# SysSec-KAIST/LTESniffer

Measured on AMD Instinct MI355X. Metric: subframes/s (20 MHz, 150 RNTIs), higher is better.
Workload: dtype f32+int16

## Files before the change

ltesniffer_amd/csrc/kernels/lsn_dsp.h:

```cpp
#pragma once
#include "lsn_dev.h"
#include "lsn_fft_map.h"

__device__ __forceinline__ cf32 cmul(cf32 a, cf32 b) { cf32 c; c.r = a.r * b.r - a.i * b.i; c.i = a.r * b.i + a.i * b.r; return c; }
__device__ __forceinline__ cf32 cmulconj(cf32 a, cf32 b) { cf32 c; c.r = a.r * b.r + a.i * b.i; c.i = a.i * b.r - a.r * b.i; return c; }
__device__ __forceinline__ float cabs2(cf32 a) { return a.r * a.r + a.i * a.i; }

template <int R, int S, int LG>
__device__ __forceinline__ void fft_twiddles(cf32* tw, const cf32* __restrict__ W, int low)
{
#pragma unroll
  for (int q = 0; q < R; q++)
#pragma unroll
    for (int m = 0; m < (1 << q); m++) tw[(1 << q) - 1 + m] = W[lsn_fft_twiddle(low + (m << S), S + q, LG)];
}
template <int R>
__device__ __forceinline__ void fft_butterflies(cf32* e, const cf32* tw)
{
#pragma unroll
  for (int q = 0; q < R; q++) {
#pragma unroll
    for (int j = 0; j < (1 << R); j++) {
      if (j & (1 << q)) continue;
      cf32 v = cmul(e[j + (1 << q)], tw[(1 << q) - 1 + (j & ((1 << q) - 1))]);
      cf32 uu = e[j];
      e[j].r = uu.r + v.r; e[j].i = uu.i + v.i;
      e[j + (1 << q)].r = uu.r - v.r; e[j + (1 << q)].i = uu.i - v.i;
    }
  }
}
template <int R, int S, int LG, int NB>
__device__ __forceinline__ void fft_pass(cf32* a, const cf32* __restrict__ W, int tid)
{
  constexpr int G = 1 << R, NG = NB << (LG - R);
#pragma unroll
  for (int u = 0; u < (NG + LSN_FFT_THREADS - 1) / LSN_FFT_THREADS; u++) {
    const int gg = tid + LSN_FFT_THREADS * u;
    if (gg < NG) {
      const int r = NB == 1 ? 0 : gg >> (LG - R), g = gg & ((1 << (LG - R)) - 1), base = lsn_fft_base(g, S, R);
      const int at = lsn_fft_store(r, base, LG);
      cf32 e[G], tw[G - 1];
#pragma unroll
      for (int j = 0; j < G; j++) e[j] = a[at ^ lsn_fft_slot(j << S)];
      fft_twiddles<R, S, LG>(tw, W, base & ((1 << S) - 1));
      fft_butterflies<R>(e, tw);
#pragma unroll
      for (int j = 0; j < G; j++) a[at ^ lsn_fft_slot(j << S)] = e[j];
    }
  }
}
template <int R, int LG>
__device__ __forceinline__ void fft_last_pass(cf32* a, const cf32* __restrict__ W, cf32* __restrict__ out, float* pw, int nre, int dc, int tid)
{
  constexpr int G = 1 << R, S = LG - R, NG = 1 << S, U = (NG + LSN_FFT_THREADS - 1) / LSN_FFT_THREADS;
  cf32 e[U][G], tw[U][G - 1];
#pragma unroll
  for (int u = 0; u < U; u++) {
    const int g = tid + LSN_FFT_THREADS * u;
    if (g < NG) {
      const int at = lsn_fft_store(0, g, LG);
#pragma unroll
      for (int j = 0; j < G; j++) e[u][j] = a[at ^ lsn_fft_slot(j << S)];
      fft_twiddles<R, S, LG>(tw[u], W, g);
    }
  }
  if (pw) __syncthreads();
#pragma unroll
  for (int u = 0; u < U; u++) {
    const int g = tid + LSN_FFT_THREADS * u;
    if (g < NG) {
      fft_butterflies<R>(e[u], tw[u]);
#pragma unroll
      for (int j = 0; j < G; j++) {
        const int k = lsn_fft_carrier(g + (j << S), 1 << LG, nre, dc);
        if (k >= 0) {
          out[k] = e[u][j];
          if (pw) pw[k] = e[u][j].r * e[u][j].r + e[u][j].i * e[u][j].i;
        }
      }
    }
  }
}
template <int LG, int NB, typename Load>
__device__ __forceinline__ void fft_run(const LsnCellDev& c, cf32* a, Load load, cf32* __restrict__ out, float* pw, int dc, int tid)
{
  constexpr int M = 1 << LG, N = NB * M;
  const cf32* __restrict__ W = c.twiddle;
  const int nre = (int)c.nre;
  if (tid < N / 8) {
    cf32 x[8], e[8], tw[7];
#pragma unroll
    for (int jj = 0; jj < 8; jj++) x[jj] = load(lsn_fft_first_sample(tid, jj, N));
#pragma unroll
    for (int j = 0; j < 8; j++) e[j] = x[lsn_fft_brev3(j)];
    fft_twiddles<3, 0, LG>(tw, W, 0);
    fft_butterflies<3>(e, tw);
    int r, g;
    lsn_fft_first_group(tid, NB, LG, &r, &g);
    const int at = lsn_fft_store(r, 8 * g, LG);
#pragma unroll
    for (int j = 0; j < 8; j++) a[at ^ lsn_fft_slot(j)] = e[j];
  }
  __syncthreads();
  constexpr int R1 = LG >= 6 ? 3 : LG - 3, S2 = 3 + R1, R2 = LG - S2 >= 3 ? 3 : LG - S2, S3 = S2 + R2, R3 = LG - S3;
  static_assert(LG >= 7 && LG <= 11 && R2 >= 1 && R3 >= 0 && R3 <= 2, "pass plan");
  static_assert(R1 == 3 && (R3 == 0 || R2 == 3), "pass plan");
  fft_pass<R1, 3, LG, NB>(a, W, tid);
  __syncthreads();
  if constexpr (R3 > 0) {
    fft_pass<R2, S2, LG, NB>(a, W, tid);
    __syncthreads();
  }
  constexpr int RL = R3 > 0 ? R3 : R2, SL = LG - RL;
  if constexpr (NB == 1) {
    fft_last_pass<RL, LG>(a, W, out, pw, nre, dc, tid);
  } else {
    fft_pass<RL, SL, LG, NB>(a, W, tid);
    __syncthreads();
    const cf32* __restrict__ T = c.twiddle3;
    float p[6];
#pragma unroll
    for (int it = 0; it < 6; it++) {
      const int k = tid + LSN_FFT_THREADS * it;
      if (k < nre) {
        const int bin = lsn_fft_carrier_bin(k, N, nre, dc), kq = bin & (M - 1);
        int b2 = 2 * bin;
        b2 = b2 >= N ? b2 - N : b2;
// ... 59 lines not shown
```

ltesniffer_amd/csrc/kernels/lsn_fft_map.h:

```cpp
#pragma once
#include <stdint.h>
#ifndef LSN_HD
#ifdef __HIPCC__
#define LSN_HD __host__ __device__ __forceinline__
#else
#define LSN_HD static inline
#endif
#endif

#define LSN_FFT_THREADS 256

LSN_HD int lsn_fft_radix(int lgM, int s) { return (s == 0 || lgM - s >= 3) ? 3 : lgM - s; }

LSN_HD int lsn_fft_first_sample(int t, int jj, int N) { return t + (N >> 3) * jj; }
LSN_HD int lsn_fft_brev3(int j) { return ((j & 1) << 2) | (j & 2) | ((j >> 2) & 1); }
LSN_HD void lsn_fft_first_group(int t, int nb, int lgM, int* r, int* g)
{
  const int tt = nb == 3 ? t / 3 : t;
  *r = nb == 3 ? t - 3 * tt : 0;
#if defined(__has_builtin) && __has_builtin(__builtin_bitreverse32)
  *g = (int)(__builtin_bitreverse32((uint32_t)tt) >> (35 - lgM));
#else
  int b = 0;
  for (int k = 0; k < lgM - 3; k++) b |= ((tt >> k) & 1) << (lgM - 4 - k);
  *g = b;
#endif
}

LSN_HD int lsn_fft_groups(int nb, int lgM, int R) { return nb << (lgM - R); }
LSN_HD int lsn_fft_base(int g, int s, int R) { return ((g >> s) << (s + R)) | (g & ((1 << s) - 1)); }
LSN_HD int lsn_fft_twiddle(int pos, int stage, int lgM) { return pos << (lgM - stage - 1); }

LSN_HD int lsn_fft_slot(int i) { return i ^ ((i >> 3) & 0x1C) ^ ((i >> 5) & 2) ^ ((i >> 7) & 0xF); }
LSN_HD int lsn_fft_block_key(int r) { return (0x1A20 >> (5 * r)) & 31; }
LSN_HD int lsn_fft_store(int r, int i, int lgM) { return (r << lgM) | (lsn_fft_slot(i) ^ lsn_fft_block_key(r)); }
LSN_HD int lsn_fft_lds_slots(int N) { return N; }

LSN_HD int lsn_fft_carrier(int bin, int N, int nre, int dc)
{
  const int hf = nre >> 1;
  if (bin >= N - hf) return bin - (N - hf);
  if (bin >= dc && bin < dc + hf) return bin - dc + hf;
  return -1;
}
LSN_HD int lsn_fft_carrier_bin(int k, int N, int nre, int dc) { return k < (nre >> 1) ? N - (nre >> 1) + k : k - (nre >> 1) + dc; }
LSN_HD void lsn_fft_last_owner(int bin, int lgM, int R, int* t, int* u, int* j)
{
  const int g = bin & ((1 << (lgM - R)) - 1);
  *j = bin >> (lgM - R);
  *t = g & (LSN_FFT_THREADS - 1);
  *u = g >> 8;
}
```

ltesniffer_amd/csrc/kernels/stage_a.hip:

```cpp
#include "lsn_dsp.h"
#include <algorithm>
#include <type_traits>
#include <cstdlib>

#define SQRT2F 1.41421356237309504880f

__device__ __forceinline__ void ofdm_rb_power(const LsnCellDev& c, const float* pw, float* __restrict__ rbp_part, int sf, int l, int tid)
{
  __syncthreads();
  if (tid < (int)c.nof_prb) {
    const float4* q = (const float4*)(pw + tid * 12);
    const float4 q0 = q[0], q1 = q[1], q2 = q[2];
    const float v[12] = {q0.x, q0.y, q0.z, q0.w, q1.x, q1.y, q1.z, q1.w, q2.x, q2.y, q2.z, q2.w};
    float s = 0.0f;
    for (int k = 0; k < 12; k++) s = s + v[k];
    rbp_part[((size_t)sf * 14 + l) * 128 + tid] = s / 12.0f;
  }
}
__global__ __launch_bounds__(256) void k_ofdm(LsnCellDev c, const cf32* __restrict__ iq, const uint32_t* __restrict__ dphi_sf,
                                              cf32* __restrict__ grid, float* __restrict__ rbp_part)
{
  extern __shared__ __attribute__((aligned(16))) unsigned char smem[];
  const int N = (int)c.N, tid = threadIdx.x;
  cf32* a = (cf32*)smem;
  const int nsym = (int)c.nsym;
  const int blk = blockIdx.x, l = blk % nsym, rx = (blk / nsym) % (int)c.nof_rx, sf = blk / (nsym * (int)c.nof_rx);
  const int cp0 = 160 * N / 2048, cp1 = 144 * N / 2048;
  const int slot = l / 7, ls = l % 7;
  const int pos = c.cp ? l * (N + N / 4) + N / 4 : slot * (cp0 + 6 * cp1 + 7 * N) + cp0 + ls * (N + cp1);
  const cf32* in = iq + ((size_t)sf * c.iq_nant + rx) * c.sflen + pos;
  const uint32_t dphi = dphi_sf ? dphi_sf[sf] : 0u;
  const int nre = (int)c.nre;
  cf32* out = grid + (((size_t)sf * c.nof_rx + rx) * 14 + l) * nre;
  auto load = [&](int n) {
    cf32 x = in[n];
    if (dphi != 0u) {
      uint32_t ph = (uint32_t)(pos + n) * dphi;
      cf32 rot = cmul(c.nco_coarse[ph >> 20], c.nco_fine[(ph >> 10) & 1023u]);
      x = cmul(x, rot);
    }
    return x;
  };
  float* pw = (rbp_part && rx == 0) ? (float*)smem : nullptr;
  lsn_symbol_fft(c, a, load, out, pw, 1, tid);
  if (pw) ofdm_rb_power(c, pw, rbp_part, sf, l, tid);
}

void lsn_launch_ofdm(const LsnCellDev& c, const cf32* iq, const uint32_t* dphi, cf32* grid, uint32_t nsf, hipStream_t s, float* rbp_part)
{
  size_t lds = sizeof(cf32) * lsn_fft_lds_slots((int)c.N);
  LSN_LAUNCH(k_ofdm, dim3(nsf * c.nof_rx * c.nsym), dim3(256), lds, s, c, iq, dphi, grid, rbp_part);
}

__device__ __forceinline__ int crs_koff(const LsnCellDev& c, int port, int s)
{
  int v = (port == 0) ? ((s & 1) ? 3 : 0) : (port == 1) ? ((s & 1) ? 0 : 3) : (port == 2) ? 3 * s : 3 + 3 * s;
  return (v + (int)(c.id % 6)) % 6;
}

__global__ __launch_bounds__(256) void k_chest(LsnCellDev c, const cf32* __restrict__ grid, const uint32_t* __restrict__ sf_idx_arr,
                                               cf32* __restrict__ ce, float* __restrict__ raw)
{
  extern __shared__ __attribute__((aligned(16))) unsigned char smem[];
  const int nre = (int)c.nre, nref = (int)c.nref, tid = threadIdx.x;
  const int P = (int)c.nof_ports, A = (int)c.nof_rx;
  const int blk = blockIdx.x, p = blk % P, rx = (blk / P) % A, sf = blk / (P * A);
  cf32* ls = (cf32*)smem;
  cf32* sm = ls + 4 * nref;
  float* part = (float*)(sm + 4 * nref);
  const int S = p < 2 ? 4 : 2;
  const int nsl = (int)c.nslot, nsym = (int)c.nsym;
  const int sym[4] = {p < 2 ? 0 : 1, p < 2 ? nsl - 3 : nsl + 1, nsl, 2 * nsl - 3};
  const cf32* g = grid + ((size_t)sf * A + rx) * 14 * nre;
  const cf32* crs = c.crs + ((size_t)sf_idx_arr[sf] * P + p) * 4 * nref;
  const int n4 = S * nref;
  for (int i = tid; i < n4; i += 256) {
    int s = i / nref, m = i - s * nref;
    ls[i] = cmulconj(g[sym[s] * nre + 6 * m + crs_koff(c, p, s)], crs[i]);
  }
  __syncthreads();
  for (int i = tid; i < n4; i += 256) {
    int s = i / nref, m = i - s * nref;
    float ar = 0.0f, ai = 0.0f;
#pragma unroll
    for (int j = 0; j < 5; j++) {
      int q = m + j - 2;
      if (q < 0 || q >= nref) continue;
      ar = ar + c.taps[j] * ls[s * nref + q].r;
      ai = ai + c.taps[j] * ls[s * nref + q].i;
    }
    sm[i].r = ar; sm[i].i = ai;
  }
  __syncthreads();
  float p0 = 0.0f, p1 = 0.0f, p2 = 0.0f, p3 = 0.0f, p4 = 0.0f, p5 = 0.0f;
  for (int i = tid; i < n4; i += 256) {
    float dr = sm[i].r - ls[i].r, di = sm[i].i - ls[i].i;
    p0 = p0 + (dr * dr + di * di);
    p1 = p1 + ls[i].r;
    p2 = p2 + ls[i].i;
    p3 = p3 + (sm[i].r * sm[i].r + sm[i].i * sm[i].i);
  }
  if (p < 2)
    for (int i = tid; i < 2 * nref; i += 256) {
      cf32 t = (i < nref) ? cmulconj(ls[2 * nref + i], ls[i]) : cmulconj(ls[3 * nref + (i - nref)], ls[nref + (i - nref)]);
      p4 = p4 + t.r;
      p5 = p5 + t.i;
    }
  part[0 * 256 + tid] = p0; part[1 * 256 + tid] = p1; part[2 * 256 + tid] = p2;
  part[3 * 256 + tid] = p3; part[4 * 256 + tid] = p4; part[5 * 256 + tid] = p5;
  __syncthreads();
  for (int s = 128; s > 0; s >>= 1) {
    if (tid < s) {
#pragma unroll
      for (int q = 0; q < 6; q++) part[q * 256 + tid] = part[q * 256 + tid] + part[q * 256 + tid + s];
    }
    __syncthreads();
  }
  if (tid < 6) raw[(((size_t)sf * A + rx) * P + p) * 8 + tid] = part[tid * 256];
  cf32* co = ce + (((size_t)sf * P + p) * A + rx) * 14 * nre;
  for (int k = tid; k < nre; k += 256) {
    cf32 row[4];
#pragma unroll
    for (int s = 0; s < 4; s++) {
      if (s >= S) break;
      int koff = crs_koff(c, p, s);
      const cf32* pl = sm + s * nref;
      int m = (k - koff) >= 0 ? (k - koff) / 6 : 0;
      if (m > nref - 2) m = nref - 2;
      float dr = (pl[m + 1].r - pl[m].r) / 6.0f, di = (pl[m + 1].i - pl[m].i) / 6.0f;
      float f = (float)(k - (6 * m + koff));
      row[s].r = pl[m].r + dr * f;
      row[s].i = pl[m].i + di * f;
    }
    if (p >= 2) {
      const cf32 c1 = row[0], c8 = row[1];
      const int la = sym[0], lb = sym[1];
      const float dl = (float)(lb - la);
      const float dr = (c8.r - c1.r) / dl, di = (c8.i - c1.i) / dl;
      co[la * nre + k] = c1; co[lb * nre + k] = c8;
      for (int l = 0; l < nsym; l++) {
        if (l == la || l == lb) continue;
        cf32 v; v.r = c1.r + dr * (float)(l - la); v.i = c1.i + di * (float)(l - la); co[l * nre + k] = v;
      }
      continue;
    }
    cf32 c0 = row[0], c4 = row[1], c7 = row[2], c11 = row[3];
    const int q0 = sym[0], q1 = sym[1], q2 = sym[2], q3 = sym[3];
    const float w01 = (float)(q1 - q0), w12 = (float)(q2 - q1), w23 = (float)(q3 - q2);
    float d01r = (c4.r - c0.r) / w01, d01i = (c4.i - c0.i) / w01;
    float d12r = (c7.r - c4.r) / w12, d12i = (c7.i - c4.i) / w12;
    float d23r = (c11.r - c7.r) / w23, d23i = (c11.i - c7.i) / w23;
    co[q0 * nre + k] = c0; co[q1 * nre + k] = c4; co[q2 * nre + k] = c7; co[q3 * nre + k] = c11;
    for (int l = q0 + 1; l < q1; l++) { cf32 v; v.r = c0.r + d01r * (float)(l - q0); v.i = c0.i + d01i * (float)(l - q0); co[l * nre + k] = v; }
    for (int l = q1 + 1; l < q2; l++) { cf32 v; v.r = c4.r + d12r * (float)(l - q1); v.i = c4.i + d12i * (float)(l - q1); co[l * nre + k] = v; }
    for (int l = q2 + 1; l < q3; l++) { cf32 v; v.r = c7.r + d23r * (float)(l - q2); v.i = c7.i + d23i * (float)(l - q2); co[l * nre + k] = v; }
    for (int l = q3 + 1; l < nsym; l++) { cf32 v; v.r = c11.r + d23r * (float)(l - q3); v.i = c11.i + d23i * (float)(l - q3); co[l * nre + k] = v; }
  }
}

void lsn_launch_chest(const LsnCellDev& c, const cf32* grid, const uint32_t* sf_idx, cf32* ce, float* raw, uint32_t nsf, hipStream_t s)
{
  size_t lds = sizeof(cf32) * 8 * c.nref + sizeof(float) * 6 * 256;
  LSN_LAUNCH(k_chest, dim3(nsf * c.nof_rx * c.nof_ports), dim3(256), lds, s, c, grid, sf_idx, ce, raw);
}

__global__ void k_chest_fin(LsnCellDev c, const float* __restrict__ raw, LsnChest* __restrict__ out, uint32_t nsf)
{
  uint32_t sf = blockIdx.x * blockDim.x + threadIdx.x;
  if (sf >= nsf) return;
  const int A = (int)c.nof_rx, P = (int)c.nof_ports;
  LsnChest o;
  float ns = 0.0f, rs = 0.0f, cp = 0.0f, cr = 0.0f, ci = 0.0f;
  for (int q = 0; q < LSN_MAX_RX * LSN_MAX_PORTS; q++) { o.noise[q] = 0.0f; o.rsrp[q] = 0.0f; o.cepow[q] = 0.0f; }
  for (int rx = 0; rx < A; rx++)
    for (int p = 0; p < P; p++) {
      const float* r = raw + (((size_t)sf * A + rx) * P + p) * 8;
      const float n = (float)((p < 2 ? 4 : 2) * c.nref);
      float noise = r[0] / n, mr = r[1] / n, mi = r[2] / n, cepow = r[3] / n;
      float rsrp = mr * mr + mi * mi;
      o.noise[rx * P + p] = noise; o.rsrp[rx * P + p] = rsrp; o.cepow[rx * P + p] = cepow;
      ns = ns + noise; rs = rs + rsrp; cp = cp + cepow;
      cr = cr + r[4]; ci = ci + r[5];
    }
  float cnt = (float)(A * P);
  o.noise_avg = ns / cnt; o.rsrp_avg = rs / cnt; o.chan_ref = cp; o.corr_r = cr; o.corr_i = ci;
  o.pad[0] = o.pad[1] = o.pad[2] = 0.0f;
  out[sf] = o;
}
void lsn_launch_chest_fin(const LsnCellDev& c, const float* raw, LsnChest* out, uint32_t nsf, hipStream_t s)
{
  LSN_LAUNCH(k_chest_fin, dim3((nsf + 63) / 64), dim3(64), 0, s, c, raw, out, nsf);
}

__device__ __forceinline__ void reg_equalise(const LsnCellDev& c, const cf32* __restrict__ g, const cf32* __restrict__ ce, float noise,
                                             int l, int k0, cf32* x, int rs, int ps)
{
  const int A = (int)c.nof_rx;
  int kk[4], n = 0;
  if ((c.reg_w6 >> l) & 1u) {
    for (int k = k0; k < k0 + 6; k++)
      if ((k % 3) != (int)(c.id % 3)) { if (n < 4) kk[n] = k; n++; }
  } else {
    for (int k = 0; k < 4; k++) kk[k] = k0 + k;
  }
  if (c.nof_ports == 1) {
#pragma unroll
    for (int i = 0; i < 4; i++) {
      float nr = 0.0f, ni = 0.0f, den = 0.0f;
      for (int rx = 0; rx < A; rx++) {
        cf32 y = g[rx * rs + kk[i]];
// ... 172 lines not shown
__device__ __forceinline__ void lsn_tb_walk4(int hw, unsigned& H)
{
  unsigned w;
  asm("v_readlane_b32 %1, %2, %0\n\ts_bitcmp1_b32 %1, %3\n\ts_addc_u32 %0, %0, %0\n\t"
      "v_readlane_b32 %1, %2, %0\n\ts_bitcmp1_b32 %1, %4\n\ts_addc_u32 %0, %0, %0\n\t"
      "v_readlane_b32 %1, %2, %0\n\ts_bitcmp1_b32 %1, %5\n\ts_addc_u32 %0, %0, %0\n\t"
      "v_readlane_b32 %1, %2, %0\n\ts_bitcmp1_b32 %1, %6\n\ts_addc_u32 %0, %0, %0"
      : "+s"(H), "=&s"(w) : "v"(hw), "n"(P), "n"(P + 1), "n"(P + 2), "n"(P + 3) : "scc");
}
__device__ __forceinline__ void viterbi_tb(const int* symw, uint32_t D_, uint32_t nbits, const uint16_t* __restrict__ crcw, int lane, unsigned long long& bits_out, uint32_t& rem_out)
{
  __syncthreads();
  const int D = (int)D_;
  const int b = lane & 1, s0 = lane >> 1;
  const int c0 = b ^ (__popc(s0 & 0x36) & 1), c1 = b ^ (__popc(s0 & 0x27) & 1), c2 = b ^ (__popc(s0 & 0x2B) & 1);
  const int signs2 = (c0 ? 0xFE : 0x02) | (c1 ? 0xFE00 : 0x0200) | (c2 ? 0xFE0000 : 0x020000);
  const int k0c = (c0 ? 127 : 128) + (c1 ? 127 : 128) + (c2 ? 127 : 128), kap = 2 * k0c - 765;
  const int pa = s0 << 2, pb = (s0 | 32) << 2;
  int m = 0;
  {
    auto step = [&](int e) {
      const int a0 = __builtin_amdgcn_ds_bpermute(pa, m) + e, a1 = __builtin_amdgcn_ds_bpermute(pb, m) - e;
      m = a1 < a0 ? a1 : a0;
    };
    int k = 0;
    for (; k + 4 <= D; k += 4) {
      int e0, e1, e2, e3;
      lsn_dot4_acc4(symw[k], symw[k + 1], symw[k + 2], symw[k + 3], signs2, kap, e0, e1, e2, e3);
      step(e0); step(e1); step(e2); step(e3);
    }
    for (; k < D; k++) step(lsn_dot4_acc(symw[k], signs2, kap));
  }
  int h2[3] = {0, 0, 0}, h3[3] = {0, 0, 0};
  auto sweep = [&](int* h) {
#pragma unroll
    for (int g = 0; g < 3; g++) {
      const int k1 = D < 32 * (g + 1) ? D : 32 * (g + 1);
      auto step = [&](int e) {
        const int a0 = __builtin_amdgcn_ds_bpermute(pa, m) + e, a1 = __builtin_amdgcn_ds_bpermute(pb, m) - e;
        lsn_push_lt(h[g], a1, a0);
        m = a1 < a0 ? a1 : a0;
      };
      int k = 32 * g;
      for (; k + 4 <= k1; k += 4) {
        int e0, e1, e2, e3;
        lsn_dot4_acc4(symw[k], symw[k + 1], symw[k + 2], symw[k + 3], signs2, kap, e0, e1, e2, e3);
        step(e0); step(e1); step(e2); step(e3);
      }
      for (; k < k1; k++) step(lsn_dot4_acc(symw[k], signs2, kap));
    }
  };
  sweep(h2);
  sweep(h3);
  unsigned long long key = ((unsigned long long)((unsigned)m ^ 0x80000000u) << 6) | (unsigned)lane;
  for (int off = 32; off > 0; off >>= 1) {
    unsigned long long o2 = __shfl_xor(key, off);
    key = o2 < key ? o2 : key;
  }
  const int rl = (int)(__brev((unsigned)lane) >> 26) << 2;
  int p2[3], p3[3];
#pragma unroll
  for (int g = 0; g < 3; g++) { p2[g] = __builtin_amdgcn_ds_bpermute(rl, h2[g]); p3[g] = __builtin_amdgcn_ds_bpermute(rl, h3[g]); }
  unsigned H = (unsigned)__builtin_amdgcn_readfirstlane((int)(__brev((unsigned)(key & 63ull)) >> 26));
  auto walk = [&](int hw, int cnt) {
    if (cnt >= 4) { lsn_tb_walk4<0>(hw, H);
    if (cnt >= 8) { lsn_tb_walk4<4>(hw, H);
    if (cnt >= 12) { lsn_tb_walk4<8>(hw, H);
    if (cnt >= 16) { lsn_tb_walk4<12>(hw, H);
    if (cnt >= 20) { lsn_tb_walk4<16>(hw, H);
    if (cnt >= 24) { lsn_tb_walk4<20>(hw, H);
    if (cnt >= 28) { lsn_tb_walk4<24>(hw, H);
    if (cnt >= 32) { lsn_tb_walk4<28>(hw, H); } } } } } } } }
    for (int p = cnt & ~3; p < cnt; p++) {
      H = (H << 1) + (((unsigned)__builtin_amdgcn_readlane(hw, (int)(H & 63u)) >> p) & 1u);
    }
  };
  int cnt[3];
#pragma unroll
  for (int g = 0; g < 3; g++) {
    const int k1 = D < 32 * (g + 1) ? D : 32 * (g + 1);
    cnt[g] = k1 > 32 * g ? k1 - 32 * g : 0;
  }
  walk(p3[2], cnt[2]); walk(p3[1], cnt[1]); walk(p3[0], cnt[0]);
  const unsigned rs0 = H & 63u;
  unsigned G[3];
#pragma unroll
  for (int g = 2; g >= 0; g--) {
    walk(p2[g], cnt[g]);
    G[g] = cnt[g] >= 32 ? H : (H & ((1u << cnt[g]) - 1u));
  }
  unsigned __int128 hb = (unsigned __int128)G[0] | ((unsigned __int128)G[1] << 32) | ((unsigned __int128)G[2] << 64) | ((unsigned __int128)rs0 << D);
  hb >>= 6;
  const unsigned long long bits = nbits ? (__brevll((unsigned long long)hb) & (~0ull << (64u - nbits))) : 0ull;
  const unsigned int tailcrc = __brev((unsigned)(hb >> nbits) & 0xFFFFu) >> 16;
  {
    unsigned int v = (lane < (int)nbits && ((bits >> (63 - lane)) & 1ull)) ? (unsigned int)crcw[lane] : 0u;
    for (int off = 32; off > 0; off >>= 1) v ^= __shfl_xor(v, off);
    rem_out = (tailcrc ^ v) & 0xFFFFu;
  }
  bits_out = bits;
}


__device__ __forceinline__ bool lsn_in_intervals(const uint32_t* iv, uint32_t n, uint32_t r)
{
  bool hit = false;
  for (uint32_t i = 0; i < n && i < 4u; i++) hit = hit || (r >= (iv[i] & 0xFFFFu) && r <= (iv[i] >> 16));
  return hit;
}
__device__ __forceinline__ uint32_t lsn_cand_claim(const LsnPruneCfg& pc, const uint32_t* __restrict__ snap, uint32_t sz, unsigned long long bits, uint32_t rnti, uint32_t ss)
{
  if (ss == 0u || rnti > 0xFFFFu) return 0u;
  const uint32_t primary = snap[2048];
  const bool active = (snap[rnti >> 5] >> (rnti & 31u)) & 1u;
  uint32_t claim = 0;
  for (uint32_t f = 0; f < 9u; f++) {
    if (pc.fmt_size[f] != sz) continue;
    if ((f == 0u || f == 2u) && ((bits >> 63) == 0ull) != (f == 0u)) continue;
    if (f == 4u && rnti > 0x000Au && rnti < 0xFFFEu) continue;
    if (rnti > 0x0001u && rnti < 0x000Au && f != 2u && f != 4u) continue;
    const bool valid = lsn_in_intervals(pc.ever[f], pc.n_ever[f], rnti) || (!lsn_in_intervals(pc.forb[f], pc.n_forb[f], rnti) && active);
    if (!valid) continue;
    claim |= ((primary >> f) & 1u) ? (ss == 1u ? 1u : 2u) : (ss == 1u ? 4u : 8u);
  }
  return claim;
}

__global__ __launch_bounds__(64) void k_viterbi(LsnCellDev c, const float* __restrict__ llr, const float* __restrict__ pw,
                                                const uint32_t* __restrict__ cfi_arr, const uint32_t* __restrict__ sf_idx_arr,
                                                LsnCand* __restrict__ cand, uint32_t* __restrict__ cand4, LsnPruneCfg pc, const uint32_t* __restrict__ snap, uint8_t* __restrict__ acc, int level,
                                                uint32_t one_sf, uint32_t one_li, uint32_t one_sz)
{
  __shared__ __attribute__((aligned(16))) int symw[LSN_MAX_DCI_D + 4];
  const int lane = threadIdx.x, sf = level == -2 ? (int)one_sf : (int)blockIdx.z, sz = (int)blockIdx.y;
  const uint32_t ncce_tot = c.nof_cce[cfi_arr[sf] - 1];
  const uint32_t lim = ncce_tot < LSN_MAX_NUM_OF_CCE ? ncce_tot : LSN_MAX_NUM_OF_CCE;
  int li, L = -1; uint32_t ncce = 0;
  if (level >= 0) {
    const uint32_t cnt = lim >> level, nloc = (lim >> 3) + (lim >> 2) + (lim >> 1) + lim;
    uint32_t off = 0, spare = 0;
    for (int l = 3; l > level; l--) { off += lim >> l; spare += (LSN_MAX_NUM_OF_CCE >> l) - (lim >> l); }
    if (blockIdx.x < cnt) { li = (int)(off + blockIdx.x); L = level; ncce = (blockIdx.x % (ncce_tot >> level)) << level; }
    else { li = (int)(nloc + spare + (blockIdx.x - cnt)); if (li >= LSN_MAX_LOC) return; }
  } else if (level == -2) {
    const int bl = blockIdx.x == 0 ? 3 : (blockIdx.x < 3 ? 2 : (blockIdx.x < 7 ? 1 : 0));
    const uint32_t j = blockIdx.x - ((1u << (3 - bl)) - 1u);
    const uint32_t idx = (one_li << (3 - bl)) + j;
    if (idx >= (lim >> bl)) return;
    uint32_t off = 0;
    for (int l = 3; l > bl; l--) off += lim >> l;
    li = (int)(off + idx); L = bl; ncce = idx << bl;
// ... 23 lines not shown
  }
  if (pc.on && level >= 0 && L < 3) {
    const uint32_t primary = snap[2048];
    bool has_p = false, has_s = false;
    for (uint32_t f = 0; f < 9u; f++)
      if (pc.fmt_size[f] == (uint32_t)sz) { if ((primary >> f) & 1u) has_p = true; else has_s = true; }
    bool closed_p = false, closed_s = false;
    uint32_t offA = 0;
    for (int la = 3; la > L; la--) {
      const uint32_t idxA = ncce >> la;
      if (idxA < (lim >> la)) {
        const unsigned long long w = *(const unsigned long long*)(acc + ((size_t)sf * LSN_MAX_LOC + offA + idxA) * LSN_MAX_SIZES);
        uint32_t m = (uint32_t)(w | (w >> 32));
        m |= m >> 16; m |= m >> 8;
        const bool first_half = ((ncce >> (la - 1)) & 1u) == 0u;
        if ((m & 3u) && (first_half || !(m & 1u))) closed_p = true;
        if (m & 3u) closed_s = true;
      }
      offA += lim >> la;
    }
    if (!((has_p && !closed_p) || (has_s && !closed_s))) {
      if (lane == 0) { out->bits = 0; out->rnti = 0; out->flags = LSN_CAND_NOT_COMPUTED; *out4 = LSN_CAND_HOT(0ull, 0u, LSN_CAND_NOT_COMPUTED); *aout = 0; }
      return;
    }
  }
  const float* e = llr + (size_t)sf * LSN_LLR_STRIDE + ncce * 72;
  const uint32_t nbits = c.sizes[sz], D = nbits + 16, D3 = 3 * D;
  const uint16_t* rank = c.rankmap + sz * 3 * LSN_MAX_DCI_D;
  bool nz = false;
  for (uint32_t t = lane; t < D; t += 64) {
    uint32_t word = 0;
#pragma unroll
    for (uint32_t j = 0; j < 3; j++) {
      float acc = 0.0f;
      bool first = true;
      for (uint32_t k = rank[3 * t + j]; k < E; k += D3) {
        float v = e[k];
        if (v != 0.0f) nz = true;
        if (first) { acc = v; first = false; } else acc = acc + v;
      }
      float q = 127.5f + 32.0f * acc;
      q = q < 0.0f ? 0.0f : q;
      q = q > 255.0f ? 255.0f : q;
      word |= (((uint32_t)(unsigned char)q - 128u) & 0xFFu) << (8 * j);
    }
    symw[t] = (int)word;
  }
  if (__ballot(nz) == 0ull) {
    if (lane == 0) { out->bits = 0; out->rnti = 0; out->flags = 0; *out4 = 0; if (pc.on) *aout = 0; }
    return;
  }
  unsigned long long bits; uint32_t rnti;
  viterbi_tb(symw, D, nbits, c.crc16_w + sz * 64, lane, bits, rnti);
  if (lane == 0) {
    const uint32_t ss = ss_validate(ncce_tot, ncce, (uint32_t)L, sf_idx_arr[sf], rnti);
    out->bits = bits;
    out->rnti = rnti;
    out->flags = 1u | (ss << 1);
    *out4 = LSN_CAND_HOT(bits, rnti, 1u | (ss << 1));
    if (pc.on && level >= 0) *aout = (uint8_t)lsn_cand_claim(pc, snap, (uint32_t)sz, bits, rnti, ss);
  }
}
__device__ __forceinline__ int pbch_count(const LsnCellDev& c) { return c.cp ? 216 : 240; }
__device__ __forceinline__ void pbch_pos(const LsnCellDev& c, int i, int& l, int& k)
{
  const int k0 = (int)c.nre / 2 - 36, l0 = (int)c.nslot;
  int s, j;
  bool crs;
  if (i < 96) { s = i / 48; j = i % 48; crs = true; }
  else if (i < 168) { s = 2; j = i - 96; crs = false; }
  else { s = 3; j = i - 168; crs = c.cp != 0; }
  l = l0 + s;
  if (crs) {
    const int r = (int)(c.id % 3);
    const int d0 = r == 0 ? 1 : 0, d1 = r == 2 ? 1 : 2;
    k = k0 + 3 * (j >> 1) + ((j & 1) ? d1 : d0);
  } else {
    k = k0 + j;
  }
}
__global__ __launch_bounds__(256) void k_pbch_llr(LsnCellDev c, const cf32* __restrict__ g, const cf32* __restrict__ ce, const LsnChest* __restrict__ ch,
                                                  float* __restrict__ out )
{
  const int tid = threadIdx.x, nre = (int)c.nre, A = (int)c.nof_rx;
  const float noise = ch[0].noise_avg;
  const int np = pbch_count(c), E4 = 2 * np;
  if (tid < 480 - E4) out[E4 + tid] = 0.0f;
  cf32 x0, x1;
  int i0 = -1;
  if (c.nof_ports == 1) {
    if (tid < np) {
      i0 = tid;
      int l, k; pbch_pos(c, tid, l, k);
      float nr = 0.0f, ni = 0.0f, den = 0.0f;
      for (int rx = 0; rx < A; rx++) {
        const size_t b = ((size_t)rx * 14 + l) * nre + k;
        const cf32 t = cmulconj(g[b], ce[b]);
        const float hp = ce[b].r * ce[b].r + ce[b].i * ce[b].i;
        if (rx == 0) { nr = t.r; ni = t.i; den = hp; } else { nr = nr + t.r; ni = ni + t.i; den = den + hp; }
      }
      den = den + noise;
      x0.r = nr / den; x0.i = ni / den;
    }
  } else if (tid < np / 2) {
    i0 = 2 * tid;
    int l, ka, kb, l2; pbch_pos(c, i0, l, ka); pbch_pos(c, i0 + 1, l2, kb);
    float x0r = 0, x0i = 0, x1r = 0, x1i = 0, hh = 0;
    const size_t pa = (c.nof_ports == 4 && (tid & 1)) ? 1 : 0, pb = c.nof_ports == 4 ? pa + 2 : 1;
    for (int rx = 0; rx < A; rx++) {
      const size_t bg = ((size_t)rx * 14 + l) * nre;
      const size_t b0 = ((pa * (size_t)A + rx) * 14 + l) * nre, b1 = ((pb * (size_t)A + rx) * 14 + l) * nre;
      const cf32 r0 = g[bg + ka], r1 = g[bg + kb];
      const cf32 h00 = ce[b0 + ka], h01 = ce[b0 + kb], h10 = ce[b1 + ka], h11 = ce[b1 + kb];
// ... 183 lines not shown
```

ltesniffer_amd/csrc/kernels/stage_c.hip:

```cpp
#include "lsn_dsp.h"
#include <algorithm>
#include "lsn_rm.h"
#include <type_traits>

#define SQRT1_2F 0.70710678118654752440f
#define SQRT2F 1.41421356237309504880f
#define LLR_Q 180.0f

__global__ __launch_bounds__(64) void k_pdsch_prep_up(LsnCellDev c, const LsnGrantDev* __restrict__ jobs_h, LsnGrantDev* __restrict__ jobs_d, uint32_t njobs,
                                                      LsnCopySegs sg, uint16_t* __restrict__ prefix)
{
  const int lane = threadIdx.x, nprb = (int)c.nof_prb;
  if (blockIdx.x >= njobs) {
    const uint32_t w = blockIdx.x - njobs, nw = gridDim.x - njobs;
    for (uint32_t q = 0; q < sg.n; q++) {
      const uint32_t words = sg.words[q];
      const bool al = ((((uintptr_t)sg.src[q]) | ((uintptr_t)sg.dst[q])) & 15u) == 0;
      const uint32_t n16 = al ? words / 4 : 0;
      const uint4* a4 = (const uint4*)sg.src[q];
      uint4* b4 = (uint4*)sg.dst[q];
      for (uint32_t i = w * 64u + (uint32_t)lane; i < n16; i += nw * 64u) b4[i] = a4[i];
      const uint32_t* a = (const uint32_t*)sg.src[q];
      uint32_t* b = (uint32_t*)sg.dst[q];
      for (uint32_t i = n16 * 4 + w * 64u + (uint32_t)lane; i < words; i += nw * 64u) b[i] = a[i];
    }
    return;
  }
  __shared__ LsnGrantDev gs;
  constexpr int NW = (int)(sizeof(LsnGrantDev) / 4);
  static_assert(NW <= 64 && sizeof(LsnGrantDev) % 4 == 0, "one word per lane");
  if (lane < NW) {
    const uint32_t v = ((const uint32_t*)(jobs_h + blockIdx.x))[lane];
    ((uint32_t*)&gs)[lane] = v;
    ((uint32_t*)(jobs_d + blockIdx.x))[lane] = v;
  }
  __syncthreads();
  const LsnGrantDev& g = gs;
  uint16_t* pf = prefix + g.prefix_off;
  const int cls = g.sf_idx == 0 ? 0 : (g.sf_idx == 5 ? 1 : 2);
  uint32_t before = 0;
  for (int l = 0; l < 14; l++) {
    uint32_t run = 0;
    for (int base = 0; base < nprb; base += 64) {
      const int prb = base + lane;
      uint32_t v = 0;
      if (prb < nprb && l >= (int)g.l0 && ((g.prb_mask[l >= (int)c.nslot ? 1 : 0][prb >> 5] >> (prb & 31)) & 1u)) v = (uint32_t)__popc((unsigned)c.validmask[(cls * 14 + l) * nprb + prb]);
      uint32_t inc = v;
#pragma unroll
      for (int off = 1; off < 64; off <<= 1) {
        const uint32_t t = __shfl_up(inc, off);
        if (lane >= off) inc += t;
      }
      if (prb < nprb) pf[l * nprb + prb] = (uint16_t)(run + inc - v);
      run += __shfl(inc, 63);
    }
    if (lane == 0) pf[lsn_rows_sym_off((uint32_t)nprb) + l] = (uint16_t)before;
    before += run;
  }
  if (lane == 0) pf[lsn_rows_sym_off((uint32_t)nprb) + 14] = (uint16_t)before;
  uint8_t* pl = (uint8_t*)(pf + lsn_rows_list_off((uint32_t)nprb));
  for (int s = 0; s < 2; s++)
    for (int prb = lane; prb < nprb; prb += 64)
      if ((g.prb_mask[s][prb >> 5] >> (prb & 31)) & 1u) pl[s * nprb + (int)lsn_rows_ordinal(g.prb_mask[s], (uint32_t)prb)] = (uint8_t)prb;
}
void lsn_launch_pdsch_prep_up(const LsnCellDev& c, const LsnGrantDev* jobs_host, LsnGrantDev* jobs_dev, uint32_t njobs, const LsnCopySegs& sg, uint16_t* prefix, hipStream_t s)
{
  uint32_t total = 0;
  for (uint32_t q = 0; q < sg.n; q++) total += sg.words[q];
  const uint32_t ncopy = total ? std::max<uint32_t>(1u, std::min<uint32_t>((total / 4 + 63u) / 64u, 256u)) : 0u;
  LSN_LAUNCH(k_pdsch_prep_up, dim3(njobs + ncopy), dim3(64), 0, s, c, jobs_host, jobs_dev, njobs, sg, prefix);
}

__device__ __forceinline__ int lsn_cvt_sat(float r)
{
  int q;
  asm("v_cvt_i32_f32 %0, %1" : "=v"(q) : "v"(r));
  return q;
}
template <int QM>
__device__ __forceinline__ void emit_q(const LsnCellDev& c, cf32 x, float w, float inv_amp, uint32_t cinit, uint32_t idx, int16_t* __restrict__ out)
{
  float L[8];
  const float wq = w * LLR_Q;
  lsn_demod_llr(QM, x.r * inv_amp, x.i * inv_amp, L);
  const uint32_t n0 = idx * (uint32_t)QM;
  uint32_t x1w[2] = {0u, 0u}, m[8];
  const uint8_t* p1 = c.gold_x1 + n0;
  const uint32_t* p2 = c.gold_x2mask + n0;
  if (QM == 8) {
    const uint2 v = *(const uint2*)p1; x1w[0] = v.x; x1w[1] = v.y;
    const uint4 a = *(const uint4*)p2, b = *(const uint4*)(p2 + 4);
    m[0] = a.x; m[1] = a.y; m[2] = a.z; m[3] = a.w; m[4] = b.x; m[5] = b.y; m[6] = b.z; m[7] = b.w;
  } else if (QM == 6) {
    const uint16_t* h = (const uint16_t*)p1;
    x1w[0] = (uint32_t)h[0] | ((uint32_t)h[1] << 16); x1w[1] = (uint32_t)h[2];
    const uint2 a = *(const uint2*)p2, b = *(const uint2*)(p2 + 2), d = *(const uint2*)(p2 + 4);
    m[0] = a.x; m[1] = a.y; m[2] = b.x; m[3] = b.y; m[4] = d.x; m[5] = d.y;
  } else if (QM == 4) {
    x1w[0] = *(const uint32_t*)p1;
    const uint4 a = *(const uint4*)p2;
    m[0] = a.x; m[1] = a.y; m[2] = a.z; m[3] = a.w;
  } else {
    x1w[0] = (uint32_t)*(const uint16_t*)p1;
    const uint2 a = *(const uint2*)p2;
    m[0] = a.x; m[1] = a.y;
  }
  uint32_t pk[4];
#pragma unroll
  for (int b = 0; b < QM; b += 2) {
    int q[2];
#pragma unroll
    for (int h = 0; h < 2; h++) {
      const int bb = b + h;
      const uint32_t sign = ((uint32_t)__popc(m[bb] & cinit) ^ (x1w[bb >> 2] >> (8 * (bb & 3)))) << 31;
      const float v = __uint_as_float(__float_as_uint(L[bb] * wq) ^ sign);
      const int t = lsn_cvt_sat(rintf(v));
// ... 498 lines not shown
```

Measured before the change: 289,800.

## Use DPP wave reductions/scans, specialize channel interpolation, and trim FFT carrier mapping

Adds DPP-based wave reduce and prefix-scan helpers and uses them in the Viterbi end-state argmin, the CRC xor-reduce and the PDSCH prefix computation. The prefix computation now uses ballot masks, scalarized grant fields, mbcnt ordinals and reuse of the previous scan when inputs repeat. The channel estimator precomputes per-pilot slopes, unrolls per-symbol loops and specializes interpolation on the slot length. The FFT last pass checks whole output rows for carrier mapping, and twiddle address arithmetic is hoisted. This cuts shuffle and integer-divide overhead across several kernels, at the cost of more code complexity and a narrower packed Viterbi key whose range is guarded by a static_assert.

```diff
diff --git a/ltesniffer_amd/csrc/kernels/lsn_dsp.h b/ltesniffer_amd/csrc/kernels/lsn_dsp.h
--- a/ltesniffer_amd/csrc/kernels/lsn_dsp.h
+++ b/ltesniffer_amd/csrc/kernels/lsn_dsp.h
@@ -6,13 +6,42 @@
 __device__ __forceinline__ cf32 cmulconj(cf32 a, cf32 b) { cf32 c; c.r = a.r * b.r + a.i * b.i; c.i = a.i * b.r - a.r * b.i; return c; }
 __device__ __forceinline__ float cabs2(cf32 a) { return a.r * a.r + a.i * a.i; }
 
+template <int CTRL, int ROWS = 0xF>
+__device__ __forceinline__ uint32_t lsn_dpp(uint32_t old, uint32_t v)
+{
+  return (uint32_t)__builtin_amdgcn_update_dpp((int)old, (int)v, CTRL, ROWS, 0xF, false);
+}
+template <class Op>
+__device__ __forceinline__ uint32_t lsn_wave_reduce(uint32_t v, Op op)
+{
+  v = op(v, lsn_dpp<0xB1>(v, v));
+  v = op(v, lsn_dpp<0x4E>(v, v));
+  v = op(v, lsn_dpp<0x141>(v, v));
+  v = op(v, lsn_dpp<0x140>(v, v));
+  v = op(v, lsn_dpp<0x142, 0xA>(v, v));
+  v = op(v, lsn_dpp<0x143, 0xC>(v, v));
+  return (uint32_t)__builtin_amdgcn_readlane((int)v, 63);
+}
+__device__ __forceinline__ uint32_t lsn_wave_scan_add(uint32_t v)
+{
+  v += lsn_dpp<0x111>(0u, v);
+  v += lsn_dpp<0x112>(0u, v);
+  v += lsn_dpp<0x114>(0u, v);
+  v += lsn_dpp<0x118>(0u, v);
+  v += lsn_dpp<0x142, 0xA>(0u, v);
+  v += lsn_dpp<0x143, 0xC>(0u, v);
+  return v;
+}
+
 template <int R, int S, int LG>
 __device__ __forceinline__ void fft_twiddles(cf32* tw, const cf32* __restrict__ W, int low)
 {
 #pragma unroll
-  for (int q = 0; q < R; q++)
-#pragma unroll
-    for (int m = 0; m < (1 << q); m++) tw[(1 << q) - 1 + m] = W[lsn_fft_twiddle(low + (m << S), S + q, LG)];
+  for (int q = 0; q < R; q++) {
+    const cf32* __restrict__ Wq = W + (uint32_t)lsn_fft_twiddle(low, S + q, LG);
+#pragma unroll
+    for (int m = 0; m < (1 << q); m++) tw[(1 << q) - 1 + m] = Wq[lsn_fft_twiddle(m << S, S + q, LG)];
+  }
 }
 template <int R>
 __device__ __forceinline__ void fft_butterflies(cf32* e, const cf32* tw)
@@ -72,7 +101,11 @@
       fft_butterflies<R>(e[u], tw[u]);
 #pragma unroll
       for (int j = 0; j < G; j++) {
-        const int k = lsn_fft_carrier(g + (j << S), 1 << LG, nre, dc);
+        const int lo = LSN_FFT_THREADS * u + (j << S), Wd = NG < LSN_FFT_THREADS ? NG : LSN_FFT_THREADS;
+        int off;
+        const int all = lsn_fft_carrier_row(lo, lo + Wd - 1, 1 << LG, nre, dc, &off);
+        if (all == 0) continue;
+        const int k = all > 0 ? g + (j << S) + off : lsn_fft_carrier(g + (j << S), 1 << LG, nre, dc);
         if (k >= 0) {
           out[k] = e[u][j];
           if (pw) pw[k] = e[u][j].r * e[u][j].r + e[u][j].i * e[u][j].i;
diff --git a/ltesniffer_amd/csrc/kernels/lsn_fft_map.h b/ltesniffer_amd/csrc/kernels/lsn_fft_map.h
--- a/ltesniffer_amd/csrc/kernels/lsn_fft_map.h
+++ b/ltesniffer_amd/csrc/kernels/lsn_fft_map.h
@@ -43,6 +43,16 @@
   if (bin >= dc && bin < dc + hf) return bin - dc + hf;
   return -1;
 }
+LSN_HD int lsn_fft_carrier_row(int lo, int hi, int N, int nre, int dc, int* off)
+{
+  const int hf = nre >> 1;
+  *off = 0;
+  if (lo >= N - hf) { *off = -(N - hf); return 1; }
+  if (hi >= N - hf) return -1;
+  if (lo >= dc && hi < dc + hf) { *off = hf - dc; return 1; }
+  if (hi < dc || lo >= dc + hf) return 0;
+  return -1;
+}
 LSN_HD int lsn_fft_carrier_bin(int k, int N, int nre, int dc) { return k < (nre >> 1) ? N - (nre >> 1) + k : k - (nre >> 1) + dc; }
 LSN_HD void lsn_fft_last_owner(int bin, int lgM, int R, int* t, int* u, int* j)
 {
diff --git a/ltesniffer_amd/csrc/kernels/stage_a.hip b/ltesniffer_amd/csrc/kernels/stage_a.hip
--- a/ltesniffer_amd/csrc/kernels/stage_a.hip
+++ b/ltesniffer_amd/csrc/kernels/stage_a.hip
@@ -69,27 +69,33 @@
   cf32* sm = ls + 4 * nref;
   float* part = (float*)(sm + 4 * nref);
   const int S = p < 2 ? 4 : 2;
-  const int nsl = (int)c.nslot, nsym = (int)c.nsym;
+  const int nsl = (int)c.nslot;
   const int sym[4] = {p < 2 ? 0 : 1, p < 2 ? nsl - 3 : nsl + 1, nsl, 2 * nsl - 3};
   const cf32* g = grid + ((size_t)sf * A + rx) * 14 * nre;
   const cf32* crs = c.crs + ((size_t)sf_idx_arr[sf] * P + p) * 4 * nref;
   const int n4 = S * nref;
-  for (int i = tid; i < n4; i += 256) {
-    int s = i / nref, m = i - s * nref;
-    ls[i] = cmulconj(g[sym[s] * nre + 6 * m + crs_koff(c, p, s)], crs[i]);
+  const int koff[4] = {crs_koff(c, p, 0), crs_koff(c, p, 1), crs_koff(c, p, 2), crs_koff(c, p, 3)};
+#pragma unroll
+  for (int s = 0; s < 4; s++) {
+    if (s >= S) break;
+    const cf32* gs = g + sym[s] * nre + koff[s];
+    for (int m = tid; m < nref; m += 256) ls[s * nref + m] = cmulconj(gs[6 * m], crs[s * nref + m]);
   }
   __syncthreads();
-  for (int i = tid; i < n4; i += 256) {
-    int s = i / nref, m = i - s * nref;
-    float ar = 0.0f, ai = 0.0f;
-#pragma unroll
-    for (int j = 0; j < 5; j++) {
-      int q = m + j - 2;
-      if (q < 0 || q >= nref) continue;
-      ar = ar + c.taps[j] * ls[s * nref + q].r;
-      ai = ai + c.taps[j] * ls[s * nref + q].i;
-    }
-    sm[i].r = ar; sm[i].i = ai;
+#pragma unroll
+  for (int s = 0; s < 4; s++) {
+    if (s >= S) break;
+    for (int m = tid; m < nref; m += 256) {
+      float ar = 0.0f, ai = 0.0f;
+#pragma unroll
+      for (int j = 0; j < 5; j++) {
+        int q = m + j - 2;
+        if (q < 0 || q >= nref) continue;
+        ar = ar + c.taps[j] * ls[s * nref + q].r;
+        ai = ai + c.taps[j] * ls[s * nref + q].i;
+      }
+      sm[s * nref + m].r = ar; sm[s * nref + m].i = ai;
+    }
   }
   __syncthreads();
   float p0 = 0.0f, p1 = 0.0f, p2 = 0.0f, p3 = 0.0f, p4 = 0.0f, p5 = 0.0f;
@@ -109,6 +115,16 @@
   part[0 * 256 + tid] = p0; part[1 * 256 + tid] = p1; part[2 * 256 + tid] = p2;
   part[3 * 256 + tid] = p3; part[4 * 256 + tid] = p4; part[5 * 256 + tid] = p5;
   __syncthreads();
+  cf32* sl = ls;
+#pragma unroll
+  for (int s = 0; s < 4; s++) {
+    if (s >= S) break;
+    const cf32* pl = sm + s * nref;
+    for (int m = tid; m < nref - 1; m += 256) {
+      cf32 d; d.r = (pl[m + 1].r - pl[m].r) / 6.0f; d.i = (pl[m + 1].i - pl[m].i) / 6.0f;
+      sl[s * nref + m] = d;
+    }
+  }
   for (int s = 128; s > 0; s >>= 1) {
     if (tid < s) {
 #pragma unroll
@@ -118,44 +134,52 @@
   }
   if (tid < 6) raw[(((size_t)sf * A + rx) * P + p) * 8 + tid] = part[tid * 256];
   cf32* co = ce + (((size_t)sf * P + p) * A + rx) * 14 * nre;
-  for (int k = tid; k < nre; k += 256) {
-    cf32 row[4];
-#pragma unroll
-    for (int s = 0; s < 4; s++) {
-      if (s >= S) break;
-      int koff = crs_koff(c, p, s);
-      const cf32* pl = sm + s * nref;
-      int m = (k - koff) >= 0 ? (k - koff) / 6 : 0;
-      if (m > nref - 2) m = nref - 2;
-      float dr = (pl[m + 1].r - pl[m].r) / 6.0f, di = (pl[m + 1].i - pl[m].i) / 6.0f;
-      float f = (float)(k - (6 * m + koff));
-      row[s].r = pl[m].r + dr * f;
-      row[s].i = pl[m].i + di * f;
-    }
-    if (p >= 2) {
-      const cf32 c1 = row[0], c8 = row[1];
-      const int la = sym[0], lb = sym[1];
-      const float dl = (float)(lb - la);
-      const float dr = (c8.r - c1.r) / dl, di = (c8.i - c1.i) / dl;
-      co[la * nre + k] = c1; co[lb * nre + k] = c8;
-      for (int l = 0; l < nsym; l++) {
-        if (l == la || l == lb) continue;
-        cf32 v; v.r = c1.r + dr * (float)(l - la); v.i = c1.i + di * (float)(l - la); co[l * nre + k] = v;
-      }
-      continue;
-    }
-    cf32 c0 = row[0], c4 = row[1], c7 = row[2], c11 = row[3];
-    const int q0 = sym[0], q1 = sym[1], q2 = sym[2], q3 = sym[3];
-    const float w01 = (float)(q1 - q0), w12 = (float)(q2 - q1), w23 = (float)(q3 - q2);
-    float d01r = (c4.r - c0.r) / w01, d01i = (c4.i - c0.i) / w01;
-    float d12r = (c7.r - c4.r) / w12, d12i = (c7.i - c4.i) / w12;
-    float d23r = (c11.r - c7.r) / w23, d23i = (c11.i - c7.i) / w23;
-    co[q0 * nre + k] = c0; co[q1 * nre + k] = c4; co[q2 * nre + k] = c7; co[q3 * nre + k] = c11;
-    for (int l = q0 + 1; l < q1; l++) { cf32 v; v.r = c0.r + d01r * (float)(l - q0); v.i = c0.i + d01i * (float)(l - q0); co[l * nre + k] = v; }
-    for (int l = q1 + 1; l < q2; l++) { cf32 v; v.r = c4.r + d12r * (float)(l - q1); v.i = c4.i + d12i * (float)(l - q1); co[l * nre + k] = v; }
-    for (int l = q2 + 1; l < q3; l++) { cf32 v; v.r = c7.r + d23r * (float)(l - q2); v.i = c7.i + d23i * (float)(l - q2); co[l * nre + k] = v; }
-    for (int l = q3 + 1; l < nsym; l++) { cf32 v; v.r = c11.r + d23r * (float)(l - q3); v.i = c11.i + d23i * (float)(l - q3); co[l * nre + k] = v; }
-  }
+  auto interpolate = [&](auto nsl_c) {
+    constexpr int NSL = decltype(nsl_c)::value, NSYM = 2 * NSL;
+    for (int k = tid; k < nre; k += 256) {
+      cf32 row[4];
+#pragma unroll
+      for (int s = 0; s < 4; s++) {
+        if (s >= S) break;
+        const cf32* pl = sm + s * nref;
+        int m = (k - koff[s]) >= 0 ? (k - koff[s]) / 6 : 0;
+        if (m > nref - 2) m = nref - 2;
+        const cf32 d = sl[s * nref + m];
+        float f = (float)(k - (6 * m + koff[s]));
+        row[s].r = pl[m].r + d.r * f;
+        row[s].i = pl[m].i + d.i * f;
+      }
+      if (p >= 2) {
+        const cf32 c1 = row[0], c8 = row[1];
+        constexpr int la = 1, lb = NSL + 1;
+        const float dl = (float)(lb - la);
+        const float dr = (c8.r - c1.r) / dl, di = (c8.i - c1.i) / dl;
+        co[la * nre + k] = c1; co[lb * nre + k] = c8;
+#pragma unroll
+        for (int l = 0; l < NSYM; l++) {
+          if (l == la || l == lb) continue;
+          cf32 v; v.r = c1.r + dr * (float)(l - la); v.i = c1.i + di * (float)(l - la); co[l * nre + k] = v;
+        }
+        continue;
+      }
+      cf32 c0 = row[0], c4 = row[1], c7 = row[2], c11 = row[3];
+      constexpr int q0 = 0, q1 = NSL - 3, q2 = NSL, q3 = 2 * NSL - 3;
+      const float w01 = (float)(q1 - q0), w12 = (float)(q2 - q1), w23 = (float)(q3 - q2);
+      float d01r = (c4.r - c0.r) / w01, d01i = (c4.i - c0.i) / w01;
+      float d12r = (c7.r - c4.r) / w12, d12i = (c7.i - c4.i) / w12;
+      float d23r = (c11.r - c7.r) / w23, d23i = (c11.i - c7.i) / w23;
+      co[q0 * nre + k] = c0; co[q1 * nre + k] = c4; co[q2 * nre + k] = c7; co[q3 * nre + k] = c11;
+#pragma unroll
+      for (int l = q0 + 1; l < q1; l++) { cf32 v; v.r = c0.r + d01r * (float)(l - q0); v.i = c0.i + d01i * (float)(l - q0); co[l * nre + k] = v; }
+#pragma unroll
+      for (int l = q1 + 1; l < q2; l++) { cf32 v; v.r = c4.r + d12r * (float)(l - q1); v.i = c4.i + d12i * (float)(l - q1); co[l * nre + k] = v; }
+#pragma unroll
+      for (int l = q2 + 1; l < q3; l++) { cf32 v; v.r = c7.r + d23r * (float)(l - q2); v.i = c7.i + d23i * (float)(l - q2); co[l * nre + k] = v; }
+#pragma unroll
+      for (int l = q3 + 1; l < NSYM; l++) { cf32 v; v.r = c11.r + d23r * (float)(l - q3); v.i = c11.i + d23i * (float)(l - q3); co[l * nre + k] = v; }
+    }
+  };
+  if (nsl == 7) interpolate(std::integral_constant<int, 7>{}); else interpolate(std::integral_constant<int, 6>{});
 }
 
 void lsn_launch_chest(const LsnCellDev& c, const cf32* grid, const uint32_t* sf_idx, cf32* ce, float* raw, uint32_t nsf, hipStream_t s)
@@ -434,16 +458,13 @@
   };
   sweep(h2);
   sweep(h3);
-  unsigned long long key = ((unsigned long long)((unsigned)m ^ 0x80000000u) << 6) | (unsigned)lane;
-  for (int off = 32; off > 0; off >>= 1) {
-    unsigned long long o2 = __shfl_xor(key, off);
-    key = o2 < key ? o2 : key;
-  }
+  static_assert(765 * 3 * LSN_MAX_DCI_D < (1 << 19), "the end-state key holds the metric in 20 bits");
+  const unsigned key = lsn_wave_reduce(((unsigned)(m + (1 << 19)) << 6) | (unsigned)lane, [](unsigned x, unsigned y) { return y < x ? y : x; });
   const int rl = (int)(__brev((unsigned)lane) >> 26) << 2;
   int p2[3], p3[3];
 #pragma unroll
   for (int g = 0; g < 3; g++) { p2[g] = __builtin_amdgcn_ds_bpermute(rl, h2[g]); p3[g] = __builtin_amdgcn_ds_bpermute(rl, h3[g]); }
-  unsigned H = (unsigned)__builtin_amdgcn_readfirstlane((int)(__brev((unsigned)(key & 63ull)) >> 26));
+  unsigned H = __brev(key & 63u) >> 26;
   auto walk = [&](int hw, int cnt) {
     if (cnt >= 4) { lsn_tb_walk4<0>(hw, H);
     if (cnt >= 8) { lsn_tb_walk4<4>(hw, H);
@@ -477,8 +498,7 @@
   const unsigned int tailcrc = __brev((unsigned)(hb >> nbits) & 0xFFFFu) >> 16;
   {
     unsigned int v = (lane < (int)nbits && ((bits >> (63 - lane)) & 1ull)) ? (unsigned int)crcw[lane] : 0u;
-    for (int off = 32; off > 0; off >>= 1) v ^= __shfl_xor(v, off);
-    rem_out = (tailcrc ^ v) & 0xFFFFu;
+    rem_out = (tailcrc ^ lsn_wave_reduce(v, [](unsigned x, unsigned y) { return x ^ y; })) & 0xFFFFu;
   }
   bits_out = bits;
 }
@@ -608,13 +628,16 @@
   }
   unsigned long long bits; uint32_t rnti;
   viterbi_tb(symw, D, nbits, c.crc16_w + sz * 64, lane, bits, rnti);
+  const uint32_t ss = ss_validate(ncce_tot, ncce, (uint32_t)L, sf_idx_arr[sf], rnti);
+  const uint32_t flags = 1u | (ss << 1);
+  const bool claimed = pc.on && level >= 0;
+  const uint32_t claim = claimed ? lsn_cand_claim(pc, snap, (uint32_t)sz, bits, rnti, ss) : 0u;
   if (lane == 0) {
-    const uint32_t ss = ss_validate(ncce_tot, ncce, (uint32_t)L, sf_idx_arr[sf], rnti);
     out->bits = bits;
     out->rnti = rnti;
-    out->flags = 1u | (ss << 1);
-    *out4 = LSN_CAND_HOT(bits, rnti, 1u | (ss << 1));
-    if (pc.on && level >= 0) *aout = (uint8_t)lsn_cand_claim(pc, snap, (uint32_t)sz, bits, rnti, ss);
+    out->flags = flags;
+    *out4 = LSN_CAND_HOT(bits, rnti, flags);
+    if (claimed) *aout = (uint8_t)claim;
   }
 }
 __device__ __forceinline__ int pbch_count(const LsnCellDev& c) { return c.cp ? 216 : 240; }
diff --git a/ltesniffer_amd/csrc/kernels/stage_c.hip b/ltesniffer_amd/csrc/kernels/stage_c.hip
--- a/ltesniffer_amd/csrc/kernels/stage_c.hip
+++ b/ltesniffer_amd/csrc/kernels/stage_c.hip
@@ -36,32 +36,60 @@
   }
   __syncthreads();
   const LsnGrantDev& g = gs;
-  uint16_t* pf = prefix + g.prefix_off;
-  const int cls = g.sf_idx == 0 ? 0 : (g.sf_idx == 5 ? 1 : 2);
+  uint16_t* pf = prefix + (uint32_t)__builtin_amdgcn_readfirstlane((int)g.prefix_off);
+  const uint32_t sfi = (uint32_t)__builtin_amdgcn_readfirstlane((int)g.sf_idx);
+  const int cls = sfi == 0 ? 0 : (sfi == 5 ? 1 : 2);
+  static_assert(sizeof(LsnGrantDev::prb_mask) == 2 * 16, "a slot mask has 128 bits: two rounds of 64 lanes cover the band");
+  const uint16_t* vm = c.validmask + cls * 14 * nprb;
+  unsigned long long am[2][2];
+  bool alloc[2][2];
+  uint32_t pv[2], pinc[2];
+#pragma unroll
+  for (int r = 0; r < 2; r++) {
+    pv[r] = 255u; pinc[r] = 0u;
+    const int left = nprb - 64 * r;
+    const unsigned long long in_band = left >= 64 ? ~0ull : (left > 0 ? (1ull << left) - 1ull : 0ull);
+#pragma unroll
+    for (int s = 0; s < 2; s++) {
+      const uint32_t lo = (uint32_t)__builtin_amdgcn_readfirstlane((int)g.prb_mask[s][2 * r]), hi = (uint32_t)__builtin_amdgcn_readfirstlane((int)g.prb_mask[s][2 * r + 1]);
+      am[s][r] = (((unsigned long long)hi << 32) | lo) & in_band;
+      alloc[s][r] = __builtin_amdgcn_inverse_ballot_w64(am[s][r]);
+    }
+  }
+  const uint32_t l0 = (uint32_t)__builtin_amdgcn_readfirstlane((int)g.l0);
   uint32_t before = 0;
+  uint32_t bl = 0;
+#pragma nounroll
   for (int l = 0; l < 14; l++) {
     uint32_t run = 0;
-    for (int base = 0; base < nprb; base += 64) {
-      const int prb = base + lane;
+    const bool s1 = l >= (int)c.nslot, on = l >= (int)l0;
+#pragma unroll
+    for (int r = 0; r < 2; r++) {
+      if (64 * r >= nprb) break;
+      const int prb = 64 * r + lane;
       uint32_t v = 0;
-      if (prb < nprb && l >= (int)g.l0 && ((g.prb_mask[l >= (int)c.nslot ? 1 : 0][prb >> 5] >> (prb & 31)) & 1u)) v = (uint32_t)__popc((unsigned)c.validmask[(cls * 14 + l) * nprb + prb]);
-      uint32_t inc = v;
-#pragma unroll
-      for (int off = 1; off < 64; off <<= 1) {
-        const uint32_t t = __shfl_up(inc, off);
-        if (lane >= off) inc += t;
-      }
+      if (__builtin_amdgcn_inverse_ballot_w64(on ? (s1 ? am[1][r] : am[0][r]) : 0ull)) v = (uint32_t)__popc((unsigned)vm[l * nprb + prb]);
+      if (__ballot(v != pv[r]) != 0ull) { pv[r] = v; pinc[r] = lsn_wave_scan_add(v); }
+      const uint32_t inc = pinc[r];
       if (prb < nprb) pf[l * nprb + prb] = (uint16_t)(run + inc - v);
-      run += __shfl(inc, 63);
-    }
-    if (lane == 0) pf[lsn_rows_sym_off((uint32_t)nprb) + l] = (uint16_t)before;
+      run += (uint32_t)__builtin_amdgcn_readlane((int)inc, 63);
+    }
+    bl = lane == l ? before : bl;
     before += run;
   }
-  if (lane == 0) pf[lsn_rows_sym_off((uint32_t)nprb) + 14] = (uint16_t)before;
+  bl = lane == 14 ? before : bl;
+  if (lane < 15) pf[lsn_rows_sym_off((uint32_t)nprb) + lane] = (uint16_t)bl;
   uint8_t* pl = (uint8_t*)(pf + lsn_rows_list_off((uint32_t)nprb));
-  for (int s = 0; s < 2; s++)
-    for (int prb = lane; prb < nprb; prb += 64)
-      if ((g.prb_mask[s][prb >> 5] >> (prb & 31)) & 1u) pl[s * nprb + (int)lsn_rows_ordinal(g.prb_mask[s], (uint32_t)prb)] = (uint8_t)prb;
+#pragma unroll
+  for (int s = 0; s < 2; s++) {
+    const uint32_t mk[4] = {(uint32_t)am[s][0], (uint32_t)(am[s][0] >> 32), (uint32_t)am[s][1], (uint32_t)(am[s][1] >> 32)};
+#pragma unroll
+    for (int r = 0; r < 2; r++) {
+      if (64 * r >= nprb) break;
+      const uint32_t ord = lsn_rows_ordinal(mk, 64u * r) + __builtin_amdgcn_mbcnt_hi((uint32_t)(am[s][r] >> 32), __builtin_amdgcn_mbcnt_lo((uint32_t)am[s][r], 0u));
+      if (alloc[s][r]) pl[s * nprb + (int)ord] = (uint8_t)(64 * r + lane);
+    }
+  }
 }
 void lsn_launch_pdsch_prep_up(const LsnCellDev& c, const LsnGrantDev* jobs_host, LsnGrantDev* jobs_dev, uint32_t njobs, const LsnCopySegs& sg, uint16_t* prefix, hipStream_t s)
 {
```

After: 288,700, median of 2. About the same (-0.4%).
